# RoyiAvital/QuadraticProgramSolver

Measured on AMD Instinct MI355X. Metric: ADMM iterations/sec, higher is better.
Workload: dtype f64

## Files before the change

quadraticprogramsolver_amd/csrc/k_loop.hip:

```cpp
#include <cstdlib>

#include "qps_kernels.h"
#include "wave_reduce.h"
#include <hip/hip_ext.h>

namespace qps {

namespace {

template <typename T> __device__ __forceinline__ T wave_sum(T v) { return wave_sum_all(v); }
__device__ __forceinline__ unsigned long long absbits(double v) { return (unsigned long long)__double_as_longlong(fabs(v)); }
__device__ __forceinline__ unsigned long long wave_max_u64(unsigned long long v) {
#pragma unroll
    for (int o = 32; o > 0; o >>= 1) { unsigned long long t = __shfl_xor(v, o, 64); v = t > v ? t : v; }
    return v;
}

template <typename T, int RB, int TRI, int THREADS>
__global__ __launch_bounds__(THREADS) void k_gemv_rows(const T* __restrict__ S, int64_t ld, const T* __restrict__ v,
                                                   T* __restrict__ out, const T* __restrict__ out0, T alpha, T beta,
                                                   int r0, int c0, int c1, BatchStride bs) {
    using V = typename VecOf<T>::type;
    if (bs.active && !bs.active[blockIdx.y]) return;
    S += (int64_t)blockIdx.y * bs.mat; v += (int64_t)blockIdx.y * bs.vin; out += (int64_t)blockIdx.y * bs.vout;
// ... 49 lines not shown
}

constexpr int GC_RT = 32;
template <typename T>
__global__ __launch_bounds__(256) void k_gemv_cols(const T* __restrict__ S, int64_t ld, const T* __restrict__ va,
                                                   const T* __restrict__ vb, T ca, T cb, T* __restrict__ part,
                                                   int64_t part_ld, int ncols) {
    using V = typename VecOf<T>::type;
    constexpr int VN = VecOf<T>::N;
    const int c = (blockIdx.x * 256 + threadIdx.x) * VN;
    if (c >= ncols) return;
    const int rt = blockIdx.y;
    const int rbase = rt * GC_RT;
    T acc[VN];
#pragma unroll
    for (int e = 0; e < VN; ++e) acc[e] = T(0);
    const T* Sp = S + (int64_t)rbase * ld + c;
#pragma unroll 8
    for (int i = 0; i < GC_RT; ++i) {
        T w = ca * va[rbase + i];
        if (vb) w += cb * vb[rbase + i];
        typedef T NV __attribute__((ext_vector_type(VN)));
        const NV a = __builtin_nontemporal_load(reinterpret_cast<const NV*>(Sp + (int64_t)i * ld));
#pragma unroll
        for (int e = 0; e < VN; ++e) acc[e] += a[e] * w;
    }
    V o;
    T* op = reinterpret_cast<T*>(&o);
#pragma unroll
    for (int e = 0; e < VN; ++e) op[e] = acc[e];
    *reinterpret_cast<V*>(part + (int64_t)rt * part_ld + c) = o;
}

template <typename T>
__global__ __launch_bounds__(256) void k_colsum(const T* __restrict__ part, int64_t part_ld, int ntiles,
                                                const T* __restrict__ a0, T s0, const T* __restrict__ a1, T s1,
                                                T* __restrict__ out, int ncols, BatchStride bs) {
    using V = typename VecOf<T>::type;
    constexpr int VN = VecOf<T>::N;
    if (bs.active && !bs.active[blockIdx.y]) return;
    part += (int64_t)blockIdx.y * bs.mat; out += (int64_t)blockIdx.y * bs.vout;
    if (a0) a0 += (int64_t)blockIdx.y * bs.vin;
    if (a1) a1 += (int64_t)blockIdx.y * bs.vin;
    constexpr int COLS = 128 / (int)sizeof(T);
    constexpr int CL = COLS / VN;
    constexpr int TL = 256 / CL;
    const int cl = threadIdx.x % CL, tl = threadIdx.x / CL;
    const int c = blockIdx.x * COLS + cl * VN;
    T acc[VN];
#pragma unroll
    for (int e = 0; e < VN; ++e) acc[e] = T(0);
    if (c < ncols) {
        int t = tl;
        for (; t + 7 * TL < ntiles; t += 8 * TL) {
            V v[8];
#pragma unroll
            for (int j = 0; j < 8; ++j) v[j] = *reinterpret_cast<const V*>(part + (int64_t)(t + TL * j) * part_ld + c);
#pragma unroll
            for (int j = 0; j < 8; ++j) {
                const T* vp = reinterpret_cast<const T*>(&v[j]);
#pragma unroll
                for (int e = 0; e < VN; ++e) acc[e] += vp[e];
            }
        }
        for (; t < ntiles; t += TL) {
            const V v = *reinterpret_cast<const V*>(part + (int64_t)t * part_ld + c);
            const T* vp = reinterpret_cast<const T*>(&v);
#pragma unroll
            for (int e = 0; e < VN; ++e) acc[e] += vp[e];
        }
    }
    __shared__ T red[TL][COLS + 1];
#pragma unroll
    for (int e = 0; e < VN; ++e) red[tl][cl * VN + e] = acc[e];
    __syncthreads();
    constexpr int PL = 256 / COLS;
    static_assert(TL % PL == 0 && (PL == 16 || PL == 8), "slab lanes per output");
    const int o = threadIdx.x / PL, pl = threadIdx.x % PL;
    T s = T(0);
#pragma unroll
    for (int k = 0; k < TL / PL; ++k) s += red[pl * (TL / PL) + k][o];
    s = (PL == 16) ? row16_sum_last(s) : oct_sum_all(s);
    const int oc = blockIdx.x * COLS + o;
    if (pl == PL - 1 && oc < ncols) {
        T r = s;
        if (a0) r += s0 * a0[oc];
        if (a1) r += s1 * a1[oc];
        out[oc] = r;
    }
}

template <typename T>
__global__ __launch_bounds__(256) void k_admm_update(int NP, int MP, const T* __restrict__ xx, const T* __restrict__ zz,
                                                     T* __restrict__ x, T* __restrict__ xp, T* __restrict__ z,
                                                     T* __restrict__ zp, T* __restrict__ y, const T* __restrict__ l,
                                                     const T* __restrict__ u, T alpha, T rho) {
    const int i = blockIdx.x * 256 + threadIdx.x;
    const T alpha1 = T(1) - alpha, rho1 = T(1) / rho;
    if (i < NP) {
        const T xo = x[i];
        xp[i] = xo;
        x[i] = alpha * xx[i] + alpha1 * xo;
    }
    if (i < MP) {
        const T zo = z[i], yo = y[i], zt = zz[i];
        zp[i] = zo;
        T t = alpha * zt + alpha1 * zo + rho1 * yo;
        const T lo = l[i], hi = u[i];
        const T zn = t > hi ? hi : (t < lo ? lo : t);
        z[i] = zn;
        y[i] = yo + rho * (alpha * zt + alpha1 * zo - zn);
    }
}

template <typename T>
__global__ __launch_bounds__(256) void k_check_norms(int n, int m, const T* __restrict__ Ax, const T* __restrict__ Px,
                                                     const T* __restrict__ Aty, const T* __restrict__ q,
// ... 3 lines not shown
    if (bs.active && !bs.active[blockIdx.y]) return;
    {
        const int64_t on = (int64_t)blockIdx.y * bs.vin, om = (int64_t)blockIdx.y * bs.vout;
        Ax += om; z += om; zp += om; Px += on; Aty += on; q += on; x += on; xp += on; slots += (int64_t)blockIdx.y * 16;
    }
    unsigned long long v[9];
#pragma unroll
    for (int k = 0; k < 9; ++k) v[k] = 0ull;
    for (int i = blockIdx.x * 256 + threadIdx.x; i < max(n, m); i += gridDim.x * 256) {
        if (i < m && !dual_only) {
            const double ax = (double)Ax[i], zi = (double)z[i];
            v[0] = max(v[0], absbits((double)(Ax[i] - z[i])));
            v[2] = max(v[2], absbits(ax));
            v[3] = max(v[3], absbits(zi));
            v[8] = max(v[8], absbits((double)(z[i] - zp[i])));
        }
        if (i < n) {
            v[1] = max(v[1], absbits((double)(Px[i] + q[i] + Aty[i])));
            v[4] = max(v[4], absbits((double)Px[i]));
            v[5] = max(v[5], absbits((double)Aty[i]));
            v[6] = max(v[6], absbits((double)q[i]));
            if (!dual_only) v[7] = max(v[7], absbits((double)(x[i] - xp[i])));
        }
    }
#pragma unroll
    for (int k = 0; k < 9; ++k) {
        v[k] = wave_max_u64(v[k]);
        if ((threadIdx.x & 63) == 0 && v[k] != 0ull) atomicMax(&slots[k], v[k]);
    }
}

__device__ __forceinline__ double jmax(double a, double b) { return (isnan(a) || isnan(b)) ? (double)NAN : (a > b ? a : b); }

__global__ void k_check_decide(const unsigned long long* __restrict__ slots, double* __restrict__ res, CheckScalars cs,
                               const double* __restrict__ rho_arr, const double* __restrict__ rhorho_arr,
                               const int* __restrict__ active) {
    if (threadIdx.x != 0) return;
    const int b = blockIdx.x;
    if (active && !active[b]) return;
    slots += (int64_t)b * 16; res += (int64_t)b * 8;
    if (rho_arr) { cs.rho = rho_arr[b]; cs.rhorho = rhorho_arr[b]; cs.convFlag = 1; }
    double nv[9];
    for (int k = 0; k < 9; ++k) nv[k] = __longlong_as_double((long long)slots[k]);
    const double MIN_VAL_RHO = 1e-3, MAX_VAL_RHO = 1e6;
    const double normResPrim = nv[0], normResDual = nv[1];
    const double maxNormPrim = jmax(nv[2], nv[3]);
    const double maxNormDual = jmax(jmax(nv[4], nv[5]), nv[6]);
    double rhorho = cs.rhorho;
    if (cs.adptRho) {
        const double numeratorVal = normResPrim * maxNormDual;
        const double denominatorVal = normResDual * maxNormPrim;
        const double t = cs.rho * sqrt(numeratorVal / denominatorVal);
        rhorho = t > MAX_VAL_RHO ? MAX_VAL_RHO : (t < MIN_VAL_RHO ? MIN_VAL_RHO : t);
    }
    const double epsPrim = cs.epsAbs + cs.epsRel * maxNormPrim;
    const double epsDual = cs.epsAbs + cs.epsRel * maxNormDual;
    int flag = cs.convFlag;
    if ((normResPrim < epsPrim) && (normResDual < epsDual)) flag = 3;
    if ((nv[7] <= cs.epsAdmm) && (nv[8] <= cs.epsAdmm)) flag = 2;
    res[0] = normResPrim; res[1] = normResDual; res[2] = maxNormPrim; res[3] = maxNormDual;
    res[4] = rhorho; res[5] = (double)flag; res[6] = nv[7]; res[7] = nv[8];
}

template <typename T> __global__ void k_fill(T* p, int64_t n, T v) {
    int64_t i = (int64_t)blockIdx.x * 256 + threadIdx.x;
    if (i < n) p[i] = v;
}
template <typename T> __global__ void k_convert(const double* __restrict__ s, T* __restrict__ d, int64_t n) {
    int64_t i = (int64_t)blockIdx.x * 256 + threadIdx.x;
    if (i < n) d[i] = (T)s[i];
}
template <typename T> __global__ void k_convert_back(const T* __restrict__ s, double* __restrict__ d, int64_t n) {
    int64_t i = (int64_t)blockIdx.x * 256 + threadIdx.x;
    if (i < n) d[i] = (double)s[i];
}

}

static int env_int(const char* name, int dflt) { const char* e = getenv(name); return e ? atoi(e) : dflt; }

template <typename T, int RB, int TH>
static void gemv_rows_launch(hipStream_t st, const T* S, int64_t ld, const T* v, T* out, const T* out0, T alpha, T beta, int r0,
                             int r1, int c0, int c1, int tri, BatchStride bs) {
    dim3 grid((r1 - r0 + RB - 1) / RB, bs.count);
#define QPS_GR(TRI) hipLaunchKernelGGL((k_gemv_rows<T, RB, TRI, TH>), grid, dim3(TH), 0, st, S, ld, v, out, out0, alpha, beta, r0, c0, c1, bs)
    if (tri == 0) QPS_GR(0); else if (tri == 1) QPS_GR(1); else QPS_GR(2);
#undef QPS_GR
}

template <typename T>
void gemv_rows(hipStream_t st, const T* S, int64_t ld, const T* v, T* out, const T* out0, T alpha, T beta, int r0, int r1,
               int c0, int c1, int tri, BatchStride bs) {
    if (r1 <= r0) return;
    static const int wide_th = env_int("QPS_GEMV_WIDE_THREADS", 512);
// ... 23 lines not shown
template <typename T>
void colsum(hipStream_t st, const T* part, int64_t part_ld, int ntiles, const T* a0, T s0, const T* a1, T s1, T* out,
            int ncols, BatchStride bs) {
    constexpr int cols_wg = 128 / (int)sizeof(T);
    if (g_launch_timing.start) {
        const LaunchTiming lt = g_launch_timing;
        g_launch_timing = LaunchTiming();
        hipExtLaunchKernelGGL((k_colsum<T>), dim3((ncols + cols_wg - 1) / cols_wg, bs.count), dim3(256), 0, st, lt.start, lt.stop, 0, part, part_ld, ntiles, a0, s0, a1, s1, out, ncols, bs);
        return;
    }
    hipLaunchKernelGGL((k_colsum<T>), dim3((ncols + cols_wg - 1) / cols_wg, bs.count), dim3(256), 0, st, part, part_ld, ntiles, a0, s0, a1, s1, out, ncols, bs);
}

template <typename T>
void admm_update(hipStream_t st, int NP, int MP, const T* xx, const T* zz, T* x, T* xp, T* z, T* zp, T* y, const T* l,
                 const T* u, T alpha, T rho) {
    const int N = NP > MP ? NP : MP;
    hipLaunchKernelGGL((k_admm_update<T>), dim3((N + 255) / 256), dim3(256), 0, st, NP, MP, xx, zz, x, xp, z, zp, y, l, u, alpha, rho);
}

template <typename T>
void check_convergence(hipStream_t st, int n, int m, const T* Ax, const T* Px, const T* Aty, const T* q, const T* x,
                       const T* xp, const T* z, const T* zp, unsigned long long* scratch, double* res_dev, CheckScalars cs,
                       int dual_only, BatchStride bs, const double* rho_arr, const double* rhorho_arr) {
    if (!dual_only) (void)hipMemsetAsync(scratch, 0, 16 * sizeof(unsigned long long) * bs.count, st);
    const int N = n > m ? n : m;
    int blocks = (N + 255) / 256;
    if (blocks > 1024) blocks = 1024;
    if (blocks < 1) blocks = 1;
    hipLaunchKernelGGL((k_check_norms<T>), dim3(blocks, bs.count), dim3(256), 0, st, n, m, Ax, Px, Aty, q, x, xp, z, zp, scratch, dual_only, bs);
    hipLaunchKernelGGL(k_check_decide, dim3(bs.count), dim3(64), 0, st, scratch, res_dev, cs, rho_arr, rhorho_arr, bs.active);
}

template <typename T> void fill(hipStream_t st, T* p, int64_t n, T v) {
    if (n <= 0) return;
    hipLaunchKernelGGL((k_fill<T>), dim3((unsigned)((n + 255) / 256)), dim3(256), 0, st, p, n, v);
}
template <typename T> void convert_copy(hipStream_t st, const double* src, T* dst, int64_t n) {
    if (n <= 0) return;
    hipLaunchKernelGGL((k_convert<T>), dim3((unsigned)((n + 255) / 256)), dim3(256), 0, st, src, dst, n);
}
template <typename T> void convert_back(hipStream_t st, const T* src, double* dst, int64_t n) {
    if (n <= 0) return;
    hipLaunchKernelGGL((k_convert_back<T>), dim3((unsigned)((n + 255) / 256)), dim3(256), 0, st, src, dst, n);
}

#define INST(T)                                                                                                              \
    template void gemv_rows<T>(hipStream_t, const T*, int64_t, const T*, T*, const T*, T, T, int, int, int, int, int, BatchStride); \
    template int gemv_cols_partial<T>(hipStream_t, const T*, int64_t, const T*, const T*, T, T, T*, int64_t, int, int);      \
    template void colsum<T>(hipStream_t, const T*, int64_t, int, const T*, T, const T*, T, T*, int, BatchStride);            \
    template void admm_update<T>(hipStream_t, int, int, const T*, const T*, T*, T*, T*, T*, T*, const T*, const T*, T, T);   \
    template void check_convergence<T>(hipStream_t, int, int, const T*, const T*, const T*, const T*, const T*, const T*,    \
                                       const T*, const T*, unsigned long long*, double*, CheckScalars, int, BatchStride,     \
                                       const double*, const double*);                                                        \
    template void fill<T>(hipStream_t, T*, int64_t, T);                                                                      \
    template void convert_copy<T>(hipStream_t, const double*, T*, int64_t);                                                  \
    template void convert_back<T>(hipStream_t, const T*, double*, int64_t);
INST(double)
INST(float)
#undef INST

}
```

quadraticprogramsolver_amd/csrc/qps_capi.hip:

```cpp
#include "ldl_symbolic.h"
#include <atomic>
#include <memory>
#include <thread>

#include "batch_schedule.h"
#include "dense_chol.h"
#include "qps_internal.h"
#include "spmv_layout.h"
#include "qps_kernels.h"
#include "qps_polish.h"
#include "qps_proxqp.h"

using namespace qps;

namespace qps {
namespace {
constexpr size_t kPinnedBytes = 512, kRecycleBlockMax = (size_t)512 << 20;
constexpr int kRecyclePerDevice = 4;
std::mutex g_res_mu;
std::vector<HandleResources> g_res[kMaxDevices];
std::atomic<int> g_cus[kMaxDevices];
}
int current_device() { int dev = 0; if (hipGetDevice(&dev) != hipSuccess) { (void)hipGetLastError(); return 0; } return dev; }
int device_cu_count(int device) {
// ... 98 lines not shown
    T *part = nullptr, *part2 = nullptr, *sw_part = nullptr, *Ax = nullptr, *Px = nullptr, *Aty = nullptr;
    T* At = nullptr; void* small_out = nullptr; void* small_out_host = nullptr; bool small_ok = false;
    StreamLease lease; Arena arena;
    double* stage_mat = nullptr; int64_t stage_mat_count = 0;
    int pass_slabs = 0, pass_rpw = 0;
    unsigned long long* scratch = nullptr; double* res_dev = nullptr; double* res_host = nullptr; double* stage = nullptr;
    bool have_AA = false, factor_valid = false; double fac_rho = 0, fac_sigma = 0; int fac_nb = 0;
    int nb = 2048; int part_tiles = 0; int num_factorizations = 0;
    unsigned long long* pub = nullptr; unsigned* abort_dev = nullptr; unsigned sweep_epoch = 0; bool blocked_off = false, fac_premul = false;
    bool use_blocked() const { return !blocked_off && trsv_blocked_supported<T>(NP, nb); }
    struct IterGraph { int count; const void* xa; double rho, sigma, alpha; int nb; hipGraphExec_t exec; };
    std::vector<IterGraph> graphs;
    bool graphs_disabled = false;
    void drop_graphs() { for (auto& gr : graphs) (void)hipGraphExecDestroy(gr.exec); graphs.clear(); }
    hipGraphExec_t iter_graph(int count, T* xa, T* xb, double rho, double sigma, double alpha) {
        for (auto& gr : graphs) if (gr.count == count && gr.xa == xa && gr.rho == rho && gr.sigma == sigma && gr.alpha == alpha && gr.nb == nb) return gr.exec;
        if (graphs_disabled) return nullptr;
        if (graphs.size() >= 8) drop_graphs();
        hipGraph_t graph = nullptr; hipGraphExec_t exec = nullptr;
        if (hipStreamBeginCapture(st, hipStreamCaptureModeThreadLocal) != hipSuccess) { (void)hipGetLastError(); graphs_disabled = true; return nullptr; }
        for (int k = 0; k < count; ++k) {
            colsum<T>(st, part, NP, pass_slabs, xa, (T)sigma, q, T(-1), tt, NP);
            sweeps();
            apass<T>(st, false, A, NP, NP, MP, xx, xa, xb, z, y, l, u, (T)alpha, (T)rho, part, part2, NP, scratch);
            std::swap(xa, xb);
        }
        if (hipStreamEndCapture(st, &graph) != hipSuccess || graph == nullptr) { (void)hipGetLastError(); graphs_disabled = true; return nullptr; }
        const hipError_t e = hipGraphInstantiate(&exec, graph, nullptr, nullptr, 0);
        (void)hipGraphDestroy(graph);
        if (e != hipSuccess) { (void)hipGetLastError(); graphs_disabled = true; return nullptr; }
        graphs.push_back({count, xa, rho, sigma, alpha, nb, exec});
        return exec;
    }
    int prof_iter = 0;
    int sample_lvl(int slot) const { return (prof.level == 1 && prof_iter % 50 == slot) ? 1 : 2; }
    int cat_atw, cat_colsum, cat_fwd, cat_bwd, cat_ax, cat_upd, cat_chk, cat_pass, cat_passchk, cat_sweep, cat_xsum, cat_small;

    DenseSolver(int dev, int64_t n_, int64_t m_, int dt) {
        device = dev; n = n_; m = m_; dtype = dt;
        HIPC(hipSetDevice(device));
        NP = roundup(n, 64); MP = roundup(m, 64);
        const int64_t nn = (int64_t)NP * NP;
        part_tiles = gemv_cols_tiles(MP);
        pass_slabs = apass_plan<T>(NP, MP, &pass_rpw);
        const int slabs = std::max(std::max(part_tiles, pass_slabs), 1);
        small_ok = admm_small_supported<T>((int)n, (int)m, NP, MP);
        stage_mat_count = std::max((int64_t)n * n, (int64_t)m * n);
        if (stage_mat_count > ((int64_t)1 << 20)) stage_mat_count = 0;
        auto layout = [&](Arena& ar) {
            A = ar.take<T>((int64_t)MP * NP); P = ar.take<T>(nn); q = ar.take<T>(NP); l = ar.take<T>(MP); u = ar.take<T>(MP);
            PI = ar.take<T>(nn); AA = ar.take<T>(nn); M = ar.take<T>(nn); S = ar.take<T>(nn); tmp = ar.take<T>(nn);
            dinv = ar.take<T>((int64_t)(NP / 64) * 4096); fail = ar.take<int>(4);
            x = ar.take<T>(NP); xp = ar.take<T>(NP); xx = ar.take<T>(NP); tt = ar.take<T>(NP); yv = ar.take<T>(NP);
            z = ar.take<T>(MP); zp = ar.take<T>(MP); y = ar.take<T>(MP); zz = ar.take<T>(MP);
            part = ar.take<T>((int64_t)slabs * NP);
            part2 = ar.take<T>((int64_t)slabs * NP);
            sw_part = ar.take<T>((int64_t)std::max(sweep_fused_slabs<T>(NP), 1) * NP);
            Ax = ar.take<T>(MP); Px = ar.take<T>(NP); Aty = ar.take<T>(NP);
            scratch = ar.take<unsigned long long>(16); res_dev = ar.take<double>(16);
            pub = ar.take<unsigned long long>(trsv_blocked_pub_words<T>(NP));
            abort_dev = reinterpret_cast<unsigned*>(res_dev + 14);
            stage = ar.take<double>((int64_t)NP + 2 * (int64_t)MP + 64);
            if (small_ok) { At = ar.take<T>((int64_t)NP * MP); small_out = ar.take<double>(32); }
            if (stage_mat_count > 0) stage_mat = ar.take<double>(stage_mat_count);
        };
        layout(arena);
        st = prof.st = lease.acquire(device, arena.planned());
        HandleResources& res = lease.res;
        char* const recycled = res.block; res.block = nullptr;
        arena.commit(st, recycled, res.block_bytes);
        layout(arena);
        res_host = reinterpret_cast<double*>(res.pinned);
        small_out_host = small_ok ? reinterpret_cast<char*>(res.pinned) + 16 * sizeof(double) : nullptr;
        const double s = sizeof(T);
        cat_atw = prof.category("gemv_cols(A'w)", s * ((double)m * n + m + n));
        cat_colsum = prof.category("colsum(rhs)", s * ((double)part_tiles * n + 3.0 * n));
        cat_fwd = prof.category("trsv_forward", s * ((double)n * (n + 1) / 2 + 2.0 * n));
        cat_bwd = prof.category("trsv_backward", s * ((double)n * (n + 1) / 2 + 2.0 * n));
        cat_ax = prof.category("gemv_rows(Ax~)", s * ((double)m * n + m + n));
        cat_upd = prof.category("admm_update", s * (3.0 * n + 7.0 * m));
        cat_chk = prof.category("check_convergence", s * (2.0 * m * n + (double)n * n + 4.0 * n + 4.0 * m));
        cat_pass = prof.category("apass(fused A-pass)", s * ((double)m * n + 3.0 * n + 6.0 * m));
        cat_passchk = prof.category("apass(check variant)", s * ((double)m * n + 4.0 * n + 6.0 * m));
        cat_sweep = prof.category("sweeps(fused fwd+bwd, triangle read once)", s * ((double)n * (n + 1) / 2 + 2.0 * n + (double)sweep_fused_slabs<T>(NP) * n));
        cat_xsum = prof.category("colsum(x~ slabs)", s * ((double)sweep_fused_slabs<T>(NP) * n + n));
        cat_small = prof.category("admm_small(whole loop in one launch; bytes per iteration)", s * ((double)m * n + (double)n * n) + s * (6.0 * n + 10.0 * m));
    }
    ~DenseSolver() override {
        (void)hipSetDevice(device);
        (void)hipStreamSynchronize(st);
        trsv_blocked_forget_stream(device, st);
        drop_graphs();
        prof.release_events();
        lease.res.block = arena.base; lease.res.block_bytes = arena.bytes; arena.base = nullptr;
    }

    void upload_vec(const double* h, T* d, int64_t count) { HIPC(upload_staged<T>(st, stage, h, d, count)); }
    void download_vec(const T* d, double* h, int64_t count) { HIPC(download_staged<T>(st, stage, d, h, count)); }
    void upload_matrix(const double* h, int64_t ldh, int rows, int cols, T* d, int64_t ldd) {
        if (rows <= 0 || cols <= 0) return;
        if (stage_mat && (int64_t)rows * cols <= stage_mat_count) {
            HIPC(hipMemcpy2DAsync(stage_mat, sizeof(double) * (size_t)rows, h, sizeof(double) * (size_t)ldh, sizeof(double) * (size_t)rows, (size_t)cols, hipMemcpyHostToDevice, st));
            import_colmajor<T>(st, stage_mat, rows, rows, cols, d, ldd);
            HIPC(hipStreamSynchronize(st));
            return;
        }
        upload_matrix_panels<T>(st, device, h, ldh, rows, cols, d, ldd);
    }

    DenseChol<T> chol() const { return {st, (int)n, NP, MP, P, A, PI, AA, M, S, tmp, dinv, fail}; }
    void factorize(double rho, double sigma, bool rebuild_all) {
        const bool rebuild = rebuild_all || !have_AA;
        const DenseChol<T> c = chol();
        factor_valid = false;
        c.form(sigma, rho, rebuild, rebuild);
        have_AA = true;
        c.factor(nb, 1, use_blocked());
        char ctx[128]; snprintf(ctx, sizeof ctx, "rho=%g, sigma=%g; factorisation #%d of this handle", rho, sigma, ++num_factorizations);
        int f = 0;
        c.check("P + sigma I + rho A'A", ctx, &f);
        factor_valid = true; fac_rho = rho; fac_sigma = sigma; fac_nb = nb; fac_premul = use_blocked();
    }
    bool sweep_gave_up(bool fetched = false) {
        if (!fac_premul) return false;
        unsigned* h = reinterpret_cast<unsigned*>(res_host + 14);
        if (!fetched) {
// ... 32 lines not shown
        sweeps();
        {
            ProfScope ps(prof, cat_ax, 2);
            gemv_rows<T>(st, A, NP, xx, zz, nullptr, T(1), T(0), 0, MP, 0, NP, 0);
        }
    }

    void solve(double* xh, const qps_params& p, qps_info* info) override {
        HIPC(hipSetDevice(device));
        blocked_off = false;
        int gave_up = 0; double t_lost = 0;
        const double t_begin = now_s();
        while (solve_once(xh, p, info)) {
            ++gave_up; t_lost = now_s() - t_begin;
            const int lvl = prof.level; prof.reset(); prof.level = lvl;
        }
        if (info) { info->sweepGaveUp = gave_up; info->cgExplicit = 0; info->tLoop += t_lost; }
    }
    bool solve_once(double* xh, const qps_params& p, qps_info* info) {
        if (p.linsys != QPS_LINSYS_AUTO && p.linsys != QPS_LINSYS_CHOLESKY)
            throw QpsError(QPS_ERR_UNSUPPORTED, "dense handles offer QPS_LINSYS_CHOLESKY only (qps_create_csc with dense_path = 0 for the CG and the sparse L D L' plugins)");
        const double t0 = now_s();
        nb = pick_nb<T>(p.trsvBlock, NP);
        double rho = p.rho, sigma = p.sigma; const double alpha = p.alpha;
        const double epsAdmm = std::fmin(p.epsAbs, p.epsRel) * 1e-2;
        int convFlag = QPS_CONV_NUM_ITR;
        const bool reuse = p.reuseFactor && factor_valid && fac_rho == rho && fac_sigma == sigma && fac_nb == nb && fac_premul == use_blocked();
        if (!reuse) factorize(rho, sigma, !p.reuseFactor || !have_AA || fac_sigma != sigma);
        upload_vec(xh, x, n);
        HIPC(hipMemsetAsync(xp, 0, sizeof(T) * NP, st));
        HIPC(hipMemsetAsync(z, 0, sizeof(T) * std::max(MP, 64), st));
        HIPC(hipMemsetAsync(y, 0, sizeof(T) * std::max(MP, 64), st));
        HIPC(hipMemsetAsync(zp, 0, sizeof(T) * std::max(MP, 64), st));
        HIPC(hipStreamSynchronize(st));
        const double t1 = now_s();
        double rhorho = rho;
        int ii = 0, nref = 0; double tref = 0, resP = NAN, resD = NAN;
        if (small_ok && p.loopVariant == 0 && (NP + nb - 1) / nb == 1) {
            transpose_small<T>(st, A, NP, MP, At);
            int it = 0;
            while (it < p.numIterations) {
                {
                    ProfScope ps(prof, cat_small, 1);
                    admm_small<T>(st, (int)n, (int)m, NP, MP, it, p.numIterations, p.numItrConv, p.adptRho, rho, rhorho, sigma, alpha, p.epsAbs,
                                  p.epsRel, epsAdmm, p.fctrRho, A, At, P, S, q, l, u, x, xp, z, y, small_out);
                }
                HIPC(hipMemcpyAsync(small_out_host, small_out, admm_small_out_bytes(), hipMemcpyDeviceToHost, st));
                HIPC(hipStreamSynchronize(st));
                prof.harvest();
                int last = 0, flag = 1, need = 0; double r8[8];
                admm_small_read(small_out_host, &last, &flag, &need, r8);
                it = last; convFlag = flag; rhorho = r8[4];
                if (!std::isnan(r8[0]) || !std::isnan(r8[1])) { resP = r8[0]; resD = r8[1]; }
                if (flag != QPS_CONV_NUM_ITR) break;
                if (need && it < p.numIterations) {
                    rho = rhorho; ++nref;
                    const double ta = now_s();
                    factorize(rho, sigma, false);
                    tref += now_s() - ta;
                }
            }
            ii = it;
            const double t2s = now_s();
            PolishReport prs;
            if (p.polish) polish_dense<T>(st, n, m, NP, MP, P, A, q, l, u, y, x, part, p, &prs);
            download_vec(x, xh, n);
            if (info) {
                info->convFlag = convFlag; info->iterations = ii; info->numRefactor = nref; info->cgIterations = 0;
                info->rhoFinal = rho; info->rhoProposed = rhorho; info->resPrim = resP; info->resDual = resD;
                info->tSetup = t1 - t0; info->tLoop = t2s - t1; info->tRefactor = tref;
                info->polishFlag = prs.flag; info->polishIterations = prs.minresIterations; info->tPolish = prs.seconds;
                info->trsvBlock = nb; info->sweepVariant = 4;
            }
            return false;
        }
        const bool fused = pass_slabs > 0 && p.loopVariant != 1;
        int rhs_slabs = 0;
        static const int graph_env = [] { const char* e = getenv("QPS_GRAPH"); return e ? atoi(e) : -1; }();
        const bool use_graph = fused && prof.level == 0 && p.numItrConv >= 3 && !fac_premul && (graph_env >= 0 ? graph_env != 0 : NP <= 2048);
        for (ii = 1; ii <= p.numIterations; ++ii) {
            bool changed = false;
            if (p.adptRho && ((rhorho * p.fctrRho < rho) || (rhorho > p.fctrRho * rho))) {
                rho = rhorho; ++nref; changed = true;
                const double ta = now_s();
                factorize(rho, sigma, false);
                tref += now_s() - ta;
            }
            const bool check = (ii % p.numItrConv == 0);
            if (use_graph && !changed && !check && rhs_slabs == pass_slabs) {
                int run = std::min(p.numItrConv - ii % p.numItrConv, p.numIterations - ii + 1) & ~1;
                hipGraphExec_t ge = run >= 2 ? iter_graph(run, x, xp, rho, sigma, alpha) : nullptr;
                if (ge) {
                    HIPC(hipGraphLaunch(ge, st));
                    ii += run - 1;
                    continue;
                }
            }
            if (!fused) {
                linear_solve(rho, sigma);
                {
                    ProfScope ps(prof, cat_upd, 2);
                    admm_update<T>(st, NP, MP, xx, zz, x, xp, z, zp, y, l, u, (T)alpha, (T)rho);
                }
                if (check) {
                    ProfScope ps(prof, cat_chk, 2);
                    gemv_rows<T>(st, A, NP, x, Ax, nullptr, T(1), T(0), 0, MP, 0, NP, 0);
                    gemv_rows<T>(st, P, NP, x, Px, nullptr, T(1), T(0), 0, NP, 0, NP, 0);
                    gemv_cols_partial<T>(st, A, NP, y, nullptr, T(1), T(0), part, NP, MP, NP);
                    colsum<T>(st, part, NP, part_tiles, nullptr, T(0), nullptr, T(0), Aty, NP);
                    CheckScalars cs{p.epsAbs, p.epsRel, epsAdmm, rho, rhorho, p.adptRho, convFlag};
                    check_convergence<T>(st, (int)n, (int)m, Ax, Px, Aty, q, x, xp, z, zp, scratch, res_dev, cs);
                }
            } else {
                if (changed && rhs_slabs > 0) {
                    ProfScope ps(prof, cat_atw, 2);
                    rhs_slabs = gemv_cols_partial<T>(st, A, NP, z, y, (T)rho, T(-1), part, NP, MP, NP);
                }
                prof_iter = ii;
                {
                    ProfLaunchScope ps(prof, cat_colsum, sample_lvl(29));
                    colsum<T>(st, part, NP, rhs_slabs, x, (T)sigma, q, T(-1), tt, NP);
                }
                sweeps();
                if (check) HIPC(hipMemsetAsync(scratch, 0, 16 * sizeof(unsigned long long), st));
                {
                    const int lvl = (prof.level == 1 && (check || ii % 50 != 38)) ? 3 : 1;
                    ProfLaunchScope ps(prof, check ? cat_passchk : cat_pass, lvl);
                    apass<T>(st, check, A, NP, NP, MP, xx, x, xp, z, y, l, u, (T)alpha, (T)rho, part, part2, NP, scratch);
                }
                std::swap(x, xp);
                rhs_slabs = pass_slabs;
                if (check) {
                    ProfScope ps(prof, cat_chk, 2);
                    colsum<T>(st, part2, NP, pass_slabs, nullptr, T(0), nullptr, T(0), Aty, NP);
                    gemv_rows<T>(st, P, NP, x, Px, nullptr, T(1), T(0), 0, NP, 0, NP, 0);
                    CheckScalars cs{p.epsAbs, p.epsRel, epsAdmm, rho, rhorho, p.adptRho, convFlag};
                    check_convergence<T>(st, (int)n, (int)m, Ax, Px, Aty, q, x, xp, z, zp, scratch, res_dev, cs, 1);
                }
            }
            if (check) {
                HIPC(hipMemcpyAsync(res_host, res_dev, 15 * sizeof(double), hipMemcpyDeviceToHost, st));
                HIPC(hipStreamSynchronize(st));
                prof.harvest();
                if (sweep_gave_up(true)) return true;
                resP = res_host[0]; resD = res_host[1]; rhorho = res_host[4]; convFlag = (int)res_host[5];
                if (convFlag != QPS_CONV_NUM_ITR) break;
            }
        }
        HIPC(hipStreamSynchronize(st));
        prof.harvest();
        if (sweep_gave_up()) return true;
        const double t2 = now_s();
        PolishReport pr;
        if (p.polish) polish_dense<T>(st, n, m, NP, MP, P, A, q, l, u, y, x, part, p, &pr);
        download_vec(x, xh, n);
        if (info) {
            info->convFlag = convFlag; info->iterations = ii > p.numIterations ? p.numIterations : ii;
            info->numRefactor = nref; info->cgIterations = 0; info->rhoFinal = rho; info->rhoProposed = rhorho;
            info->resPrim = resP; info->resDual = resD; info->tSetup = t1 - t0; info->tLoop = t2 - t1; info->tRefactor = tref;
            info->polishFlag = pr.flag; info->polishIterations = pr.minresIterations; info->tPolish = pr.seconds;
            info->trsvBlock = nb; info->sweepVariant = sweep_variant();
        }
        return false;
    }
    void polish(double* xh, const double* yh, const qps_params& p, qps_polish_report* rep) override {
        HIPC(hipSetDevice(device));
        upload_vec(xh, x, n); upload_vec(yh, y, m);
        PolishReport pr;
        polish_dense<T>(st, n, m, NP, MP, P, A, q, l, u, y, x, part, p, &pr);
        download_vec(x, xh, n);
        if (rep) {
            rep->flag = pr.flag; rep->refinements = pr.refinements; rep->minresIterations = pr.minresIterations;
            rep->numActiveLower = pr.numLower; rep->numActiveUpper = pr.numUpper; rep->reserved0 = 0; rep->relres = pr.relres; rep->seconds = pr.seconds;
        }
    }
    void get_dual(double* zh, double* yh) override {
// ... 1033 lines not shown
```

quadraticprogramsolver_amd/csrc/qps_internal.h:

```cpp
#pragma once
#include <hip/hip_runtime.h>

#include <algorithm>
#include <chrono>
#include <cmath>
#include <cstdio>
#include <cstring>
#include <mutex>
#include <string>
#include <system_error>
#include <thread>
#include <vector>

#include "../../include/qps.h"

namespace qps {

struct QpsError { int code; std::string msg; QpsError(int c, std::string m) : code(c), msg(std::move(m)) {} };

inline double now_s() { return std::chrono::duration<double>(std::chrono::steady_clock::now().time_since_epoch()).count(); }
inline int roundup(int64_t v, int q) { return (int)(((v + q - 1) / q) * q); }

struct KernelStat { double seconds = 0; int64_t launches = 0; double algo_bytes = 0; };

struct Profiler {
    int level = 0;
    hipStream_t st = nullptr;
    struct Pending { int cat; hipEvent_t a, b; };
    std::vector<Pending> pending;
    std::vector<hipEvent_t> pool;
    std::vector<std::string> names;
    std::vector<KernelStat> stats;
    int category(const char* name, double bytes) {
        for (size_t i = 0; i < names.size(); ++i) if (names[i] == name) return (int)i;
        names.push_back(name); KernelStat s; s.algo_bytes = bytes; stats.push_back(s); return (int)names.size() - 1;
    }
    hipEvent_t get() { if (!pool.empty()) { hipEvent_t e = pool.back(); pool.pop_back(); return e; } hipEvent_t e; (void)hipEventCreate(&e); return e; }
    bool on(int cat_level) const { return level >= cat_level; }
    void begin(int cat, hipEvent_t& a) { a = get(); (void)hipEventRecord(a, st); (void)cat; }
    void end(int cat, hipEvent_t a) { hipEvent_t b = get(); (void)hipEventRecord(b, st); pending.push_back({cat, a, b}); }
    void harvest() {
        for (auto& p : pending) {
            float ms = 0; (void)hipEventElapsedTime(&ms, p.a, p.b);
            stats[p.cat].seconds += ms * 1e-3; stats[p.cat].launches += 1;
            pool.push_back(p.a); pool.push_back(p.b);
        }
        pending.clear();
    }
    void reset() { for (auto& s : stats) { s.seconds = 0; s.launches = 0; } }
    void release_events() {
        for (auto e : pool) (void)hipEventDestroy(e);
        for (auto& p : pending) { (void)hipEventDestroy(p.a); (void)hipEventDestroy(p.b); }
        pool.clear(); pending.clear();
    }
    ~Profiler() { for (auto e : pool) (void)hipEventDestroy(e); for (auto& p : pending) { (void)hipEventDestroy(p.a); (void)hipEventDestroy(p.b); } }
};
struct ProfLaunchScope {
    Profiler& p; int cat; hipEvent_t a, b; bool active;
    ProfLaunchScope(Profiler& pr, int c, int lvl);
    ~ProfLaunchScope();
};
struct ProfScope {
    Profiler& p; int cat; hipEvent_t a; bool active;
    ProfScope(Profiler& pr, int c, int lvl) : p(pr), cat(c), a(nullptr), active(pr.on(lvl)) { if (active) p.begin(cat, a); }
    ~ProfScope() { if (active) p.end(cat, a); }
};

#define HIPC(expr)                                                                                            \
    do {                                                                                                      \
        hipError_t e_ = (expr);                                                                               \
        if (e_ != hipSuccess) {                                                                               \
            char b_[512]; snprintf(b_, sizeof b_, "%s failed: %s (%s:%d)", #expr, hipGetErrorString(e_), __FILE__, __LINE__); \
            throw QpsError(e_ == hipErrorOutOfMemory ? QPS_ERR_OUT_OF_MEMORY : QPS_ERR_HIP, b_);               \
        }                                                                                                     \
    } while (0)

struct DeviceOwner {
    std::vector<void*> dev, host;
    DeviceOwner() = default;
    DeviceOwner(const DeviceOwner&) = delete;
// ... 152 lines not shown
```

quadraticprogramsolver_amd/csrc/qps_kernels.h:

```cpp
#pragma once
#ifndef QPS_NT_SLABS
#define QPS_NT_SLABS 1
#endif
#include <hip/hip_runtime.h>
#include <stdint.h>

#include <atomic>
#include <thread>

namespace qps {

constexpr int kMaxDevices = 64;
int current_device();
int device_cu_count(int device);
struct PerDeviceOnce {
    std::atomic<unsigned char> state[kMaxDevices] = {};
    template <typename F> void once(int dev, F&& f) {
        if (dev < 0 || dev >= kMaxDevices) { f(); return; }
        if (state[dev].load(std::memory_order_acquire) == 2) return;
        unsigned char expect = 0;
        if (state[dev].compare_exchange_strong(expect, 1, std::memory_order_acq_rel)) { f(); state[dev].store(2, std::memory_order_release); return; }
        while (state[dev].load(std::memory_order_acquire) != 2) std::this_thread::yield();
    }
};
// ... 1 lines not shown
struct LaunchTiming { hipEvent_t start = nullptr, stop = nullptr; };
extern thread_local LaunchTiming g_launch_timing;


struct BatchStride { int count = 1; int64_t mat = 0, vin = 0, vout = 0; const int* active = nullptr; };

template <typename T> struct VecOf;
template <> struct VecOf<double> { using type = double2; static constexpr int N = 2; };
template <> struct VecOf<float>  { using type = float4;  static constexpr int N = 4; };

template <typename T>
void gemv_rows(hipStream_t st, const T* S, int64_t ld, const T* v, T* out, const T* out0, T alpha, T beta,
               int r0, int r1, int c0, int c1, int tri, BatchStride bs = BatchStride());

template <typename T>
int gemv_cols_partial(hipStream_t st, const T* S, int64_t ld, const T* va, const T* vb, T ca, T cb,
                      T* part, int64_t part_ld, int nrows, int ncols);
int gemv_cols_tiles(int nrows);

template <typename T>
void colsum(hipStream_t st, const T* part, int64_t part_ld, int ntiles, const T* a0, T s0, const T* a1, T s1,
            T* out, int ncols, BatchStride bs = BatchStride());

template <typename T>
void admm_update(hipStream_t st, int NP, int MP, const T* xx, const T* zz, T* x, T* xp, T* z, T* zp, T* y,
                 const T* l, const T* u, T alpha, T rho);

struct CheckScalars { double epsAbs, epsRel, epsAdmm, rho, rhorho; int adptRho; int convFlag; };
template <typename T>
void check_convergence(hipStream_t st, int n, int m, const T* Ax, const T* Px, const T* Aty, const T* q, const T* x,
                       const T* xp, const T* z, const T* zp, unsigned long long* scratch , double* res_dev,
                       CheckScalars cs, int dual_only = 0, BatchStride bs = BatchStride(), const double* rho_arr = nullptr,
                       const double* rhorho_arr = nullptr);

template <typename T> int apass_plan(int NP, int MP, int* rows_per_wg, int count = 1);
template <typename T> int apass_max_np();
struct PassBatch { int count = 1; int slabs = 0; const double* rho_arr = nullptr; const int* active = nullptr; int pq_me = 0; };
template <typename T>
void apass(hipStream_t st, bool check, const T* A, int64_t ld, int NP, int MP, const T* xx, const T* x_old, T* x_new, T* z,
           T* y, const T* l, const T* u, T alpha, T rho, T* part, T* part2, int64_t part_ld, unsigned long long* slots,
           PassBatch pb = PassBatch());
template <typename T> int apass_proxqp_slabs(int NP, int MP);
template <typename T>
int apass_kkt(hipStream_t st, const T* A, int64_t ld, int NP, int MP, const T* vx, const T* vlam, const T* mask, T delta, T* out_lam,
              T* part, int64_t part_ld);
template <typename T>
int apass_proxqp(hipStream_t st, const T* G, int64_t ld, int NP, int MP, int me, const T* x, T* x_scratch, T* slack, T* dual,
                 const T* g, T rho, T* part, int64_t part_ld);

template <typename T> bool sweep_fused_supported(int NP);
template <typename T> int sweep_fused_slabs(int NP, int count = 1);
template <typename T>
int sweep_fused(hipStream_t st, const T* S, int64_t ld, int NP, const T* v, T* part, int64_t part_ld, BatchStride bs = BatchStride());

template <typename T> struct PanelArgs {
    const T* Mat = nullptr; int64_t ld = 0; int rows = 0, K = 0;
    const T* B = nullptr; int npanel = 0;
    T* out = nullptr;
    const T* q = nullptr; T *x = nullptr, *xp = nullptr;
    T *z = nullptr, *zp = nullptr, *y = nullptr, *w = nullptr; const T *l = nullptr, *u = nullptr;
    const int* active = nullptr;
    T alpha = T(0), rho = T(1), sigma = T(0);
};
enum class SharedPanelOp {
    product,
    rhs,
// ... 75 lines not shown
```

Measured before the change: 14590.

## Fuse convergence check tail into one kernel and overlap next iteration's front

Fuses the Aty column sum, the dual-residual max reductions and the convergence decision into a single last-block-finishes kernel that writes results straight to host-mapped memory. This removes the separate colsum, check and decide launches, the scratch memset and the device-to-host copy. It also enqueues the next iteration's colsum and sweeps before the host blocks on the check event, so GPU work continues while the host waits. In exchange it relies on grid-wide atomic arrival counting and speculatively queued work, which is discarded when rho changes.

```diff
diff --git a/quadraticprogramsolver_amd/csrc/k_loop.hip b/quadraticprogramsolver_amd/csrc/k_loop.hip
--- a/quadraticprogramsolver_amd/csrc/k_loop.hip
+++ b/quadraticprogramsolver_amd/csrc/k_loop.hip
@@ -105,19 +105,18 @@
     *reinterpret_cast<V*>(part + (int64_t)rt * part_ld + c) = o;
 }
 
-template <typename T>
-__global__ __launch_bounds__(256) void k_colsum(const T* __restrict__ part, int64_t part_ld, int ntiles,
-                                                const T* __restrict__ a0, T s0, const T* __restrict__ a1, T s1,
-                                                T* __restrict__ out, int ncols, BatchStride bs) {
+template <typename T> struct ColsumGeom {
+    static constexpr int VN = VecOf<T>::N;
+    static constexpr int COLS = 128 / (int)sizeof(T);
+    static constexpr int CL = COLS / VN;
+    static constexpr int TL = 256 / CL;
+    static constexpr int PL = 256 / COLS;
+};
+template <typename T>
+__device__ __forceinline__ T colsum_slabs(const T* __restrict__ part, int64_t part_ld, int ntiles, int ncols, int* oc, bool* last) {
     using V = typename VecOf<T>::type;
-    constexpr int VN = VecOf<T>::N;
-    if (bs.active && !bs.active[blockIdx.y]) return;
-    part += (int64_t)blockIdx.y * bs.mat; out += (int64_t)blockIdx.y * bs.vout;
-    if (a0) a0 += (int64_t)blockIdx.y * bs.vin;
-    if (a1) a1 += (int64_t)blockIdx.y * bs.vin;
-    constexpr int COLS = 128 / (int)sizeof(T);
-    constexpr int CL = COLS / VN;
-    constexpr int TL = 256 / CL;
+    using G = ColsumGeom<T>;
+    constexpr int VN = G::VN, COLS = G::COLS, CL = G::CL, TL = G::TL;
     const int cl = threadIdx.x % CL, tl = threadIdx.x / CL;
     const int c = blockIdx.x * COLS + cl * VN;
     T acc[VN];
@@ -147,15 +146,29 @@
 #pragma unroll
     for (int e = 0; e < VN; ++e) red[tl][cl * VN + e] = acc[e];
     __syncthreads();
-    constexpr int PL = 256 / COLS;
+    constexpr int PL = G::PL;
     static_assert(TL % PL == 0 && (PL == 16 || PL == 8), "slab lanes per output");
     const int o = threadIdx.x / PL, pl = threadIdx.x % PL;
     T s = T(0);
 #pragma unroll
     for (int k = 0; k < TL / PL; ++k) s += red[pl * (TL / PL) + k][o];
     s = (PL == 16) ? row16_sum_last(s) : oct_sum_all(s);
-    const int oc = blockIdx.x * COLS + o;
-    if (pl == PL - 1 && oc < ncols) {
+    *oc = blockIdx.x * COLS + o;
+    *last = (pl == PL - 1);
+    return s;
+}
+
+template <typename T>
+__global__ __launch_bounds__(256) void k_colsum(const T* __restrict__ part, int64_t part_ld, int ntiles,
+                                                const T* __restrict__ a0, T s0, const T* __restrict__ a1, T s1,
+                                                T* __restrict__ out, int ncols, BatchStride bs) {
+    if (bs.active && !bs.active[blockIdx.y]) return;
+    part += (int64_t)blockIdx.y * bs.mat; out += (int64_t)blockIdx.y * bs.vout;
+    if (a0) a0 += (int64_t)blockIdx.y * bs.vin;
+    if (a1) a1 += (int64_t)blockIdx.y * bs.vin;
+    int oc; bool last;
+    const T s = colsum_slabs<T>(part, part_ld, ntiles, ncols, &oc, &last);
+    if (last && oc < ncols) {
         T r = s;
         if (a0) r += s0 * a0[oc];
         if (a1) r += s1 * a1[oc];
@@ -225,6 +238,26 @@
 
 __device__ __forceinline__ double jmax(double a, double b) { return (isnan(a) || isnan(b)) ? (double)NAN : (a > b ? a : b); }
 
+__device__ __forceinline__ void check_decide(const double (&nv)[9], const CheckScalars& cs, double* __restrict__ res) {
+    const double MIN_VAL_RHO = 1e-3, MAX_VAL_RHO = 1e6;
+    const double normResPrim = nv[0], normResDual = nv[1];
+    const double maxNormPrim = jmax(nv[2], nv[3]);
+    const double maxNormDual = jmax(jmax(nv[4], nv[5]), nv[6]);
+    double rhorho = cs.rhorho;
+    if (cs.adptRho) {
+        const double numeratorVal = normResPrim * maxNormDual;
+        const double denominatorVal = normResDual * maxNormPrim;
+        const double t = cs.rho * sqrt(numeratorVal / denominatorVal);
+        rhorho = t > MAX_VAL_RHO ? MAX_VAL_RHO : (t < MIN_VAL_RHO ? MIN_VAL_RHO : t);
+    }
+    const double epsPrim = cs.epsAbs + cs.epsRel * maxNormPrim;
+    const double epsDual = cs.epsAbs + cs.epsRel * maxNormDual;
+    int flag = cs.convFlag;
+    if ((normResPrim < epsPrim) && (normResDual < epsDual)) flag = 3;
+    if ((nv[7] <= cs.epsAdmm) && (nv[8] <= cs.epsAdmm)) flag = 2;
+    res[0] = normResPrim; res[1] = normResDual; res[2] = maxNormPrim; res[3] = maxNormDual;
+    res[4] = rhorho; res[5] = (double)flag; res[6] = nv[7]; res[7] = nv[8];
+}
 __global__ void k_check_decide(const unsigned long long* __restrict__ slots, double* __restrict__ res, CheckScalars cs,
                                const double* __restrict__ rho_arr, const double* __restrict__ rhorho_arr,
                                const int* __restrict__ active) {
@@ -235,24 +268,54 @@
     if (rho_arr) { cs.rho = rho_arr[b]; cs.rhorho = rhorho_arr[b]; cs.convFlag = 1; }
     double nv[9];
     for (int k = 0; k < 9; ++k) nv[k] = __longlong_as_double((long long)slots[k]);
-    const double MIN_VAL_RHO = 1e-3, MAX_VAL_RHO = 1e6;
-    const double normResPrim = nv[0], normResDual = nv[1];
-    const double maxNormPrim = jmax(nv[2], nv[3]);
-    const double maxNormDual = jmax(jmax(nv[4], nv[5]), nv[6]);
-    double rhorho = cs.rhorho;
-    if (cs.adptRho) {
-        const double numeratorVal = normResPrim * maxNormDual;
-        const double denominatorVal = normResDual * maxNormPrim;
-        const double t = cs.rho * sqrt(numeratorVal / denominatorVal);
-        rhorho = t > MAX_VAL_RHO ? MAX_VAL_RHO : (t < MIN_VAL_RHO ? MIN_VAL_RHO : t);
-    }
-    const double epsPrim = cs.epsAbs + cs.epsRel * maxNormPrim;
-    const double epsDual = cs.epsAbs + cs.epsRel * maxNormDual;
-    int flag = cs.convFlag;
-    if ((normResPrim < epsPrim) && (normResDual < epsDual)) flag = 3;
-    if ((nv[7] <= cs.epsAdmm) && (nv[8] <= cs.epsAdmm)) flag = 2;
-    res[0] = normResPrim; res[1] = normResDual; res[2] = maxNormPrim; res[3] = maxNormDual;
-    res[4] = rhorho; res[5] = (double)flag; res[6] = nv[7]; res[7] = nv[8];
+    check_decide(nv, cs, res);
+}
+
+template <typename T>
+__global__ __launch_bounds__(256) void k_check_tail(const T* __restrict__ part2, int64_t part_ld, int ntiles, int ncols, int n,
+                                                    const T* __restrict__ Px, const T* __restrict__ q,
+                                                    unsigned long long* __restrict__ slots, double* __restrict__ res_host,
+                                                    const unsigned* __restrict__ abort_dev, CheckScalars cs) {
+    int oc; bool last;
+    const T aty = colsum_slabs<T>(part2, part_ld, ntiles, ncols, &oc, &last);
+    unsigned long long v[4] = {0ull, 0ull, 0ull, 0ull};
+    if (last && oc < n) {
+        const T px = Px[oc], qq = q[oc];
+        v[0] = absbits((double)(px + qq + aty));
+        v[1] = absbits((double)px);
+        v[2] = absbits((double)aty);
+        v[3] = absbits((double)qq);
+    }
+    __shared__ unsigned long long wmax[4][4];
+    __shared__ int am_last;
+#pragma unroll
+    for (int k = 0; k < 4; ++k) {
+        v[k] = wave_max_u64(v[k]);
+        if ((threadIdx.x & 63) == 0) wmax[threadIdx.x >> 6][k] = v[k];
+    }
+    __syncthreads();
+    if (threadIdx.x == 0) {
+        constexpr int slot_of[4] = {1, 4, 5, 6};
+#pragma unroll
+        for (int k = 0; k < 4; ++k) {
+            unsigned long long w = wmax[0][k];
+#pragma unroll
+            for (int j = 1; j < 4; ++j) w = wmax[j][k] > w ? wmax[j][k] : w;
+            if (w != 0ull) atomicMax(&slots[slot_of[k]], w);
+        }
+        const unsigned long long arrived = __hip_atomic_fetch_add(&slots[15], 1ull, __ATOMIC_ACQ_REL, __HIP_MEMORY_SCOPE_AGENT);
+        am_last = (arrived == (unsigned long long)gridDim.x - 1ull);
+    }
+    __syncthreads();
+    if (!am_last || threadIdx.x != 0) return;
+    double nv[9];
+    for (int k = 0; k < 9; ++k) nv[k] = __longlong_as_double((long long)__hip_atomic_load(&slots[k], __ATOMIC_RELAXED, __HIP_MEMORY_SCOPE_AGENT));
+    double res[8];
+    check_decide(nv, cs, res);
+    for (int k = 0; k < 8; ++k) res_host[k] = res[k];
+    reinterpret_cast<unsigned*>(res_host + 14)[0] = *abort_dev;
+    for (int k = 0; k < 16; ++k) __hip_atomic_store(&slots[k], 0ull, __ATOMIC_RELAXED, __HIP_MEMORY_SCOPE_AGENT);
+    __threadfence_system();
 }
 
 template <typename T> __global__ void k_fill(T* p, int64_t n, T v) {
@@ -342,6 +405,13 @@
     hipLaunchKernelGGL(k_check_decide, dim3(bs.count), dim3(64), 0, st, scratch, res_dev, cs, rho_arr, rhorho_arr, bs.active);
 }
 
+template <typename T>
+void check_tail(hipStream_t st, int n, int NP, const T* part2, int64_t part_ld, int ntiles, const T* Px, const T* q,
+                unsigned long long* slots, double* res_host, const unsigned* abort_dev, CheckScalars cs) {
+    constexpr int cols_wg = 128 / (int)sizeof(T);
+    hipLaunchKernelGGL((k_check_tail<T>), dim3((NP + cols_wg - 1) / cols_wg), dim3(256), 0, st, part2, part_ld, ntiles, NP, n, Px, q, slots, res_host, abort_dev, cs);
+}
+
 template <typename T> void fill(hipStream_t st, T* p, int64_t n, T v) {
     if (n <= 0) return;
     hipLaunchKernelGGL((k_fill<T>), dim3((unsigned)((n + 255) / 256)), dim3(256), 0, st, p, n, v);
@@ -363,6 +433,8 @@
     template void check_convergence<T>(hipStream_t, int, int, const T*, const T*, const T*, const T*, const T*, const T*,    \
                                        const T*, const T*, unsigned long long*, double*, CheckScalars, int, BatchStride,     \
                                        const double*, const double*);                                                        \
+    template void check_tail<T>(hipStream_t, int, int, const T*, int64_t, int, const T*, const T*, unsigned long long*,      \
+                                double*, const unsigned*, CheckScalars);                                                     \
     template void fill<T>(hipStream_t, T*, int64_t, T);                                                                      \
     template void convert_copy<T>(hipStream_t, const double*, T*, int64_t);                                                  \
     template void convert_back<T>(hipStream_t, const T*, double*, int64_t);
diff --git a/quadraticprogramsolver_amd/csrc/qps_capi.hip b/quadraticprogramsolver_amd/csrc/qps_capi.hip
--- a/quadraticprogramsolver_amd/csrc/qps_capi.hip
+++ b/quadraticprogramsolver_amd/csrc/qps_capi.hip
@@ -154,6 +154,7 @@
         graphs.push_back({count, xa, rho, sigma, alpha, nb, exec});
         return exec;
     }
+    hipEvent_t chk_done = nullptr;
     int prof_iter = 0;
     int sample_lvl(int slot) const { return (prof.level == 1 && prof_iter % 50 == slot) ? 1 : 2; }
     int cat_atw, cat_colsum, cat_fwd, cat_bwd, cat_ax, cat_upd, cat_chk, cat_pass, cat_passchk, cat_sweep, cat_xsum, cat_small;
@@ -214,6 +215,7 @@
         trsv_blocked_forget_stream(device, st);
         drop_graphs();
         prof.release_events();
+        if (chk_done) (void)hipEventDestroy(chk_done);
         lease.res.block = arena.base; lease.res.block_bytes = arena.bytes; arena.base = nullptr;
     }
 
@@ -312,6 +314,7 @@
         HIPC(hipMemsetAsync(z, 0, sizeof(T) * std::max(MP, 64), st));
         HIPC(hipMemsetAsync(y, 0, sizeof(T) * std::max(MP, 64), st));
         HIPC(hipMemsetAsync(zp, 0, sizeof(T) * std::max(MP, 64), st));
+        HIPC(hipMemsetAsync(scratch, 0, 16 * sizeof(unsigned long long), st));
         HIPC(hipStreamSynchronize(st));
         const double t1 = now_s();
         double rhorho = rho;
@@ -358,6 +361,15 @@
         int rhs_slabs = 0;
         static const int graph_env = [] { const char* e = getenv("QPS_GRAPH"); return e ? atoi(e) : -1; }();
         const bool use_graph = fused && prof.level == 0 && p.numItrConv >= 3 && !fac_premul && (graph_env >= 0 ? graph_env != 0 : NP <= 2048);
+        bool front_queued = false;
+        auto front = [&](int it) {
+            prof_iter = it;
+            {
+                ProfLaunchScope ps(prof, cat_colsum, sample_lvl(29));
+                colsum<T>(st, part, NP, rhs_slabs, x, (T)sigma, q, T(-1), tt, NP);
+            }
+            sweeps();
+        };
         for (ii = 1; ii <= p.numIterations; ++ii) {
             bool changed = false;
             if (p.adptRho && ((rhorho * p.fctrRho < rho) || (rhorho > p.fctrRho * rho))) {
@@ -367,7 +379,8 @@
                 tref += now_s() - ta;
             }
             const bool check = (ii % p.numItrConv == 0);
-            if (use_graph && !changed && !check && rhs_slabs == pass_slabs) {
+            if (changed) front_queued = false;
+            if (use_graph && !changed && !check && !front_queued && rhs_slabs == pass_slabs) {
                 int run = std::min(p.numItrConv - ii % p.numItrConv, p.numIterations - ii + 1) & ~1;
                 hipGraphExec_t ge = run >= 2 ? iter_graph(run, x, xp, rho, sigma, alpha) : nullptr;
                 if (ge) {
@@ -396,13 +409,9 @@
                     ProfScope ps(prof, cat_atw, 2);
                     rhs_slabs = gemv_cols_partial<T>(st, A, NP, z, y, (T)rho, T(-1), part, NP, MP, NP);
                 }
+                if (!front_queued) front(ii);
+                front_queued = false;
                 prof_iter = ii;
-                {
-                    ProfLaunchScope ps(prof, cat_colsum, sample_lvl(29));
-                    colsum<T>(st, part, NP, rhs_slabs, x, (T)sigma, q, T(-1), tt, NP);
-                }
-                sweeps();
-                if (check) HIPC(hipMemsetAsync(scratch, 0, 16 * sizeof(unsigned long long), st));
                 {
                     const int lvl = (prof.level == 1 && (check || ii % 50 != 38)) ? 3 : 1;
                     ProfLaunchScope ps(prof, check ? cat_passchk : cat_pass, lvl);
@@ -411,17 +420,26 @@
                 std::swap(x, xp);
                 rhs_slabs = pass_slabs;
                 if (check) {
-                    ProfScope ps(prof, cat_chk, 2);
-                    colsum<T>(st, part2, NP, pass_slabs, nullptr, T(0), nullptr, T(0), Aty, NP);
-                    gemv_rows<T>(st, P, NP, x, Px, nullptr, T(1), T(0), 0, NP, 0, NP, 0);
-                    CheckScalars cs{p.epsAbs, p.epsRel, epsAdmm, rho, rhorho, p.adptRho, convFlag};
-                    check_convergence<T>(st, (int)n, (int)m, Ax, Px, Aty, q, x, xp, z, zp, scratch, res_dev, cs, 1);
+                    {
+                        ProfScope ps(prof, cat_chk, 2);
+                        gemv_rows<T>(st, P, NP, x, Px, nullptr, T(1), T(0), 0, NP, 0, NP, 0);
+                        CheckScalars cs{p.epsAbs, p.epsRel, epsAdmm, rho, rhorho, p.adptRho, convFlag};
+                        check_tail<T>(st, (int)n, NP, part2, NP, pass_slabs, Px, q, scratch, res_host, abort_dev, cs);
+                    }
+                    if (!chk_done) HIPC(hipEventCreateWithFlags(&chk_done, hipEventDisableTiming));
+                    HIPC(hipEventRecord(chk_done, st));
+                    const size_t recorded = prof.pending.size();
+                    if (ii < p.numIterations && !fac_premul) { front(ii + 1); front_queued = true; }
+                    HIPC(hipEventSynchronize(chk_done));
+                    prof.harvest(recorded);
                 }
             }
             if (check) {
-                HIPC(hipMemcpyAsync(res_host, res_dev, 15 * sizeof(double), hipMemcpyDeviceToHost, st));
-                HIPC(hipStreamSynchronize(st));
-                prof.harvest();
+                if (!fused) {
+                    HIPC(hipMemcpyAsync(res_host, res_dev, 15 * sizeof(double), hipMemcpyDeviceToHost, st));
+                    HIPC(hipStreamSynchronize(st));
+                    prof.harvest();
+                }
                 if (sweep_gave_up(true)) return true;
                 resP = res_host[0]; resD = res_host[1]; rhorho = res_host[4]; convFlag = (int)res_host[5];
                 if (convFlag != QPS_CONV_NUM_ITR) break;
diff --git a/quadraticprogramsolver_amd/csrc/qps_internal.h b/quadraticprogramsolver_amd/csrc/qps_internal.h
--- a/quadraticprogramsolver_amd/csrc/qps_internal.h
+++ b/quadraticprogramsolver_amd/csrc/qps_internal.h
@@ -39,13 +39,15 @@
     bool on(int cat_level) const { return level >= cat_level; }
     void begin(int cat, hipEvent_t& a) { a = get(); (void)hipEventRecord(a, st); (void)cat; }
     void end(int cat, hipEvent_t a) { hipEvent_t b = get(); (void)hipEventRecord(b, st); pending.push_back({cat, a, b}); }
-    void harvest() {
-        for (auto& p : pending) {
+    void harvest(size_t count = (size_t)-1) {
+        count = std::min(count, pending.size());
+        for (size_t i = 0; i < count; ++i) {
+            const Pending& p = pending[i];
             float ms = 0; (void)hipEventElapsedTime(&ms, p.a, p.b);
             stats[p.cat].seconds += ms * 1e-3; stats[p.cat].launches += 1;
             pool.push_back(p.a); pool.push_back(p.b);
         }
-        pending.clear();
+        pending.erase(pending.begin(), pending.begin() + (std::ptrdiff_t)count);
     }
     void reset() { for (auto& s : stats) { s.seconds = 0; s.launches = 0; } }
     void release_events() {
diff --git a/quadraticprogramsolver_amd/csrc/qps_kernels.h b/quadraticprogramsolver_amd/csrc/qps_kernels.h
--- a/quadraticprogramsolver_amd/csrc/qps_kernels.h
+++ b/quadraticprogramsolver_amd/csrc/qps_kernels.h
@@ -57,6 +57,10 @@
                        const T* xp, const T* z, const T* zp, unsigned long long* scratch , double* res_dev,
                        CheckScalars cs, int dual_only = 0, BatchStride bs = BatchStride(), const double* rho_arr = nullptr,
                        const double* rhorho_arr = nullptr);
+
+template <typename T>
+void check_tail(hipStream_t st, int n, int NP, const T* part2, int64_t part_ld, int ntiles, const T* Px, const T* q,
+                unsigned long long* slots, double* res_host, const unsigned* abort_dev, CheckScalars cs);
 
 template <typename T> int apass_plan(int NP, int MP, int* rows_per_wg, int count = 1);
 template <typename T> int apass_max_np();
```

After: 14690, median of 6. About the same (+0.7%).
